# cafferychen777/flashdeconv

Hardware: AMD Instinct MI355X
Metric: spots/sec to convergence (1M x 2000 x 30) (higher is better)
Workload: dtype f64

## Files before the change

### flashdeconv_amd/csrc/tile_kernels.cpp

```cpp
#include "fdx_env.h"
#include <algorithm>
#include <cmath>
#include <cstdlib>
#include <memory>
#include <mutex>

#include "fdx_internal.h"
#include "fdx_kernels.h"
#include "sketch_plan.h"
#include "tile_device.h"
#include "tile_plan.h"
#include "tile_variant.h"

namespace fdx {

struct TilePlanDevice {
    TilePlanHost h;
    DevBuf w, off, len, ent_base, slot_bucket;
    int RS = 0;
    int WB = 0;
    size_t lds = 0;
};

const double* log_table_dev(hipStream_t st) {
    static std::mutex mu;
    static double* tabs[64] = {};
    int dev = 0;
    if (hipGetDevice(&dev) != hipSuccess || dev < 0 || dev >= 64) return nullptr;
    std::lock_guard<std::mutex> lock(mu);
    if (!tabs[dev]) {
        std::vector<double> t((size_t)LOG_TAB_N);
        for (int i = 0; i < LOG_TAB_N; ++i) {
            const unsigned bits = (unsigned)(LOG_TAB_BASE + i) << LOG_TAB_SHIFT;
            float c;
            std::memcpy(&c, &bits, 4);
            t[(size_t)i] = (double)(-logl((long double)c) + (long double)LOG_TAB_EXP_SHIFT * 0.693147180559945309417232121458176568L);
        }
        double* p = nullptr;
        if (hipMalloc(&p, t.size() * sizeof(double)) != hipSuccess) return nullptr;
        if (hipMemcpyAsync(p, t.data(), t.size() * sizeof(double), hipMemcpyHostToDevice, st) != hipSuccess ||
            hipStreamSynchronize(st) != hipSuccess) {
            (void)hipFree(p);
            return nullptr;
        }
        tabs[dev] = p;
    }
    return tabs[dev];
}

static thread_local bool t_f64_math = false;
TileF64Math::TileF64Math(bool on) : prev(t_f64_math) { t_f64_math = on; }
TileF64Math::~TileF64Math() { t_f64_math = prev; }

static int tile_logv() {
    if (t_f64_math) return 0;
    const char* e = fdx::env("FDX_TILE_LOGV");
    return e ? atoi(e) : 2;
}

static bool tile_cfg(int dtype, int mode, int K, int d, int logv, TileVariant* out) {
    if ((dtype != FDX_F32 && dtype != FDX_F64) || K < 1 || K > 64 || d < 1) return false;
    if (mode != FDX_PRE_RAW && mode != FDX_PRE_LOG_CPM && mode != FDX_PRE_LOG_CPM_SPARSE) return false;
    const bool raw = mode == FDX_PRE_RAW;
    TileVariant v = raw ? TileVariant{12, 4, 11} : TileVariant{16, 0, 8};
    v.TT = (K + 15) / 16;
    if (K > 32 || d > 4 * v.NWC * v.JW) {
        v = raw ? TileVariant{12, 4, 22, 4, true} : TileVariant{8, 0, 32, 4, true};
        if (d > 4 * v.NWC * v.JW) return false;
    }
    v.logv = (dtype == FDX_F32 && !raw && logv != 0) ? 2 : 0;
    v.avl2 = v.wide || (!raw && v.logv == 0);
    v.wg = v.wide && raw;
    *out = v;
    return true;
}

static size_t tile_lds_bytes(int RS, int NE, int mode, int WB = 0) {
    const size_t NEp = ((size_t)NE + 7) & ~(size_t)7;
    const size_t below = 2 * ((size_t)WB + (size_t)TILE_ROWS * RS) + NEp * (WB ? 2 : 10) + 2 * TILE_ROWS * (8 + 4);
    if (mode == FDX_PRE_RAW) return below;
    return below <= (size_t)LOG_TAB_LDS ? (size_t)160 * 1024 : (size_t)161 * 1024;
}

static const TilePlanDevice* tile_plan_for(const SketchPlan& sp, int dtype, int mode, const TileVariant& v, hipStream_t st) {
    const int sz = dtype == FDX_F32 ? 4 : 8;
    const int key = ((dtype == FDX_F32 ? 0 : 1) * 2 + (mode != FDX_PRE_RAW ? 1 : 0)) * 3 + (v.wide ? 2 : v.TT - 1);
    static_assert(SketchPlan::kTileKeys == 12, "key space of the schedules: input type x raw / log x {one tile, two tiles, wide}");
    std::lock_guard<std::mutex> lock(sp.tile_mu);
    if (sp.tile_tried[key]) return sp.tile[key].get();
    sp.tile_tried[key] = true;
    const bool dbg = fdx::env("FDX_DEBUG") != nullptr;
    if (!sp.scatter_ok || sp.host_bucket.empty()) return nullptr;
    const size_t red_bytes = tile_red_bytes(v.NWC, v.avl2, v.TT);
    const int unit = (v.wide ? 128 : 1024) / sz;
    std::unique_ptr<TilePlanDevice> best;
    int GB0 = (int)round_up(sp.G, unit);
    while ((size_t)(v.wg ? round_up((GB0 + 1) * 8, 16) : 0) + (size_t)TILE_ROWS * (GB0 * sz + TILE_ROW_PAD) < red_bytes) GB0 += unit;
    for (int GB = GB0; GB >= unit; GB -= unit) {
        const int RS = GB * sz + TILE_ROW_PAD;
        const int WB = v.wg ? (int)round_up((GB + 1) * 8, 16) : 0;
        if ((size_t)WB + (size_t)TILE_ROWS * RS < red_bytes) break;
        if (tile_lds_bytes(RS, sp.G, mode, WB) > 160 * 1024) continue;
        auto cand = std::make_unique<TilePlanDevice>();
        if (!build_tile_plan(sp.host_bucket.data(), sp.host_w.data(), sp.G, sp.d, v.NWC, v.JW, GB, &cand->h)) return nullptr;
        cand->RS = RS;
        cand->WB = WB;
        cand->lds = tile_lds_bytes(RS, cand->h.NE, mode, WB);
        if (dbg) std::fprintf(stderr, "[fdx] tile plan: G=%d d=%d waves=%d+%d GB=%d blocks=%d NE=%d steps=%d lds=%zu\n", sp.G, sp.d, v.NWC,
                              v.NWL, GB, cand->h.NBLK, cand->h.NE, cand->h.steps, cand->lds);
        if (cand->lds > 160 * 1024) continue;
        best = std::move(cand);
        break;
    }
    if (!best) return nullptr;
    TilePlanDevice& t = *best;
    auto up = [&](DevBuf& b, const void* src, size_t bytes) -> int {
        FDX_TRY(b.alloc(bytes));
        FDX_TRY(copy_h2d(b.p, src, bytes, st));
        return 0;
    };
    const int jp = JW_PAD(v.JW);
    std::vector<unsigned char> len_pad((size_t)v.NWC * t.h.NBLK * jp + 16, 0);
    for (int wv = 0; wv < v.NWC; ++wv)
        for (int c = 0; c < t.h.NBLK; ++c)
            for (int j = 0; j < v.JW; ++j)
                len_pad[((size_t)wv * t.h.NBLK + c) * jp + j] = t.h.len[((size_t)wv * t.h.NBLK + c) * v.JW + j];
    std::vector<double> wg_tab;
    if (t.WB) {
        const int per = t.WB / 8;
        wg_tab.assign((size_t)t.h.NBLK * per, 0.0);
        for (int g = 0; g < sp.G; ++g)
            if (sp.host_bucket[(size_t)g] >= 0) wg_tab[(size_t)(g / t.h.GB) * per + g % t.h.GB] = sp.host_w[(size_t)g];
        for (size_t i = 0; i < t.h.off.size(); ++i)
            if (t.h.gene[i] < 0) t.h.off[i] = (unsigned short)t.h.GB;
    }
    if ((t.WB ? up(t.w, wg_tab.data(), wg_tab.size() * 8) : up(t.w, t.h.w.data(), t.h.w.size() * 8)) ||
        up(t.off, t.h.off.data(), t.h.off.size() * 2) || up(t.len, len_pad.data(), len_pad.size()) || up(t.ent_base, t.h.ent_base.data(), t.h.ent_base.size() * 4) ||
        up(t.slot_bucket, t.h.slot_bucket.data(), t.h.slot_bucket.size() * 4))
        return nullptr;
    if (hipStreamSynchronize(st) != hipSuccess) return nullptr;
    sp.tile[key] = std::move(best);
    return sp.tile[key].get();
}

__global__ void tile_xa_kernel(const double* __restrict__ Xs, const int* __restrict__ slot_bucket, int K, int d, int n_groups,
                               int TT, double* __restrict__ XA) {
    const int i = blockIdx.x * blockDim.x + threadIdx.x;
    if (i >= n_groups * TT * 64) return;
    const int lane = i & 63, t = (i >> 6) % TT, wj = (i >> 6) / TT;
    const int b = slot_bucket[wj * 4 + (lane >> 4)];
    const int type = t * 16 + (lane & 15);
    XA[i] = (b >= 0 && type < K) ? Xs[(size_t)type * d + b] : 0.0;
}

bool tile_sketch_ok(int dtype, long long ldy, const void* Y, int G, int d, int K, int mode, const SketchPlanDev& plan,
                    hipStream_t st) {
    if (!plan.owner) return false;
    TileVariant v;
    if (G <= 0 || !tile_cfg(dtype, mode, K, d, tile_logv(), &v)) return false;
    const int sz = dtype == FDX_F32 ? 4 : 8;
    if ((K > 32 || d > 512) && fdx::env("FDX_NO_TILE_WIDE")) return false;
    if (((size_t)G * sz) % 16 != 0 || ((size_t)ldy * sz) % 16 != 0 || (reinterpret_cast<uintptr_t>(Y) & 15) != 0) return false;
    return tile_plan_for(*plan.owner, dtype, mode, v, st) != nullptr;
}

int launch_tile_sketch(const void* Y, int dtype, long long ldy, const int* row_map, long long n, int G, int d, int mode,
                       const SketchPlanDev& plan, const double* Xs, int K, double* H, long long ldh, double* row_sumsq,
                       hipStream_t st) {
    if (n <= 0) return 0;
    TileVariant v;
    const TilePlanDevice* t = plan.owner && tile_cfg(dtype, mode, K, d, tile_logv(), &v) ? tile_plan_for(*plan.owner, dtype, mode, v, st) : nullptr;
    if (!t) return fail(FDX_ERR_INVALID, "tile sketch: no schedule for this shape");
    const void* kern = dtype == FDX_F32 ? tile_kernel<float>(mode, v) : tile_kernel<double>(mode, v);
    if (!kern) {
        char msg[128];
        std::snprintf(msg, sizeof msg, "tile sketch: no kernel for dtype %d mode %d, waves %d + %d x %d, TT %d, AVL2 %d, LOGV %d, WG %d",
                      dtype, mode, v.NWC, v.NWL, v.JW, v.TT, (int)v.avl2, v.logv, (int)v.wg);
        return fail(FDX_ERR_INVALID, msg);
    }
    TileArgs a{};
    a.ldy = ldy; a.n = n; a.ldh = ldh; a.G = G; a.d = d; a.K = K;
    a.NE = t->h.NE; a.GB = t->h.GB; a.NBLK = t->h.NBLK; a.RS = t->RS; a.jw_used = t->h.jw_used; a.WB = t->WB;
    const double* w_tab = t->w.as<double>();
    const unsigned short* off_tab = t->off.as<unsigned short>();
    const unsigned char* len_tab = t->len.as<unsigned char>();
    const int* ent_base = t->ent_base.as<int>();
    const int* slot_bucket = t->slot_bucket.as<int>();
    const double* log_tab = nullptr;
    if (mode != FDX_PRE_RAW) {
        log_tab = log_table_dev(st);
        if (!log_tab) return fail(FDX_ERR_HIP, "tile sketch: log table upload failed");
    }
    const long long n_tiles = (n + TILE_ROWS - 1) / TILE_ROWS;
    const int grid = (int)std::min<long long>(n_tiles, 256);
    DevBuf xa;
    const double* XA = nullptr;
    if (v.avl2) {
        const int n_groups = v.NWC * v.JW;
        FDX_TRY(xa.alloc((size_t)n_groups * v.TT * 64 * sizeof(double)));
        hipLaunchKernelGGL(tile_xa_kernel, dim3(ceil_div((long long)n_groups * v.TT * 64, 256)), dim3(256), 0, st, Xs, slot_bucket, K, d,
                           n_groups, v.TT, xa.as<double>());
        FDX_CHECK_LAUNCH();
        XA = xa.as<double>();
    }
    if (t->lds > 64 * 1024) FDX_HIP(hipFuncSetAttribute(kern, hipFuncAttributeMaxDynamicSharedMemorySize, (int)t->lds));
    void* args[] = {(void*)&a, (void*)&Y, (void*)&row_map, (void*)&Xs, (void*)&H, (void*)&row_sumsq, (void*)&w_tab, (void*)&off_tab,
                    (void*)&len_tab, (void*)&ent_base, (void*)&slot_bucket, (void*)&log_tab, (void*)&XA};
    FDX_HIP(hipLaunchKernel(kern, dim3(grid), dim3((v.NWC + v.NWL) * 64), args, t->lds, st));
    return 0;
}

bool fused_sketch_contract_ok(int dtype, long long ldy, const void* Y, int G, int d, int K, int mode, const SketchPlanDev& plan,
                              hipStream_t st) {
    if (fdx::env("FDX_NO_FUSED")) return false;
    return tile_sketch_ok(dtype, ldy, Y, G, d, K, mode, plan, st);
}

int launch_sketch_contract(const void* Y, int dtype, long long ldy, const int* row_map, long long n, int G, int d, int mode,
                           const SketchPlanDev& plan, const double* Xs, int K, double* H, long long ldh, double* row_sumsq,
                           hipStream_t st) {
    if (n <= 0) return 0;
    if (!tile_sketch_ok(dtype, ldy, Y, G, d, K, mode, plan, st)) return fail(FDX_ERR_INVALID, "sketch -> H: no one-kernel form for this shape");
    return launch_tile_sketch(Y, dtype, ldy, row_map, n, G, d, mode, plan, Xs, K, H, ldh, row_sumsq, st);
}

}

namespace fdx {
__global__ void log1p_f32_probe_kernel(const float* __restrict__ y, float scale, long long n, float* __restrict__ out) {
    const long long i = (long long)blockIdx.x * blockDim.x + threadIdx.x;
    if (i < n) out[i] = tile_log1p_f32(y[i], scale);
}
}

extern "C" int fdx_log1p_f32(const float* y, float scale, int64_t n, float* out) {
    using namespace fdx;
    FDX_REQUIRE(n >= 0 && (n == 0 || (y && out)), "fdx_log1p_f32: null argument");
    if (n == 0) return 0;
    DevBuf in, res;
    FDX_TRY(in.alloc((size_t)n * 4));
    FDX_TRY(res.alloc((size_t)n * 4));
    FDX_HIP(hipMemcpy(in.p, y, (size_t)n * 4, hipMemcpyHostToDevice));
    hipLaunchKernelGGL(log1p_f32_probe_kernel, dim3((unsigned)ceil_div(n, 256)), dim3(256), 0, nullptr, in.as<float>(), scale,
                       (long long)n, res.as<float>());
    FDX_CHECK_LAUNCH();
    FDX_HIP(hipMemcpy(out, res.p, (size_t)n * 4, hipMemcpyDeviceToHost));
    return 0;
}

extern "C" int fdx_tile_schedule(const int32_t* gene_bucket, const double* gene_w, int32_t G, int32_t d, int32_t NW,
                                   int32_t JW, int32_t GB, int32_t* dims_out ,
                                   int32_t* slot_bucket_out, uint8_t* len_out, int32_t* ent_base_out, double* w_out,
                                   uint16_t* off_out, int64_t cap_entries) {
    using namespace fdx;
    FDX_REQUIRE(gene_bucket && gene_w && dims_out, "fdx_tile_schedule: null argument");
    TilePlanHost h;
    FDX_REQUIRE(build_tile_plan(gene_bucket, gene_w, G, d, NW, JW, GB, &h), "fdx_tile_schedule: shape cannot be scheduled");
    dims_out[0] = h.NBLK; dims_out[1] = h.NE; dims_out[2] = h.steps; dims_out[3] = h.max_wave_steps;
    if (!slot_bucket_out) return 0;
    FDX_REQUIRE(len_out && ent_base_out && w_out && off_out && cap_entries >= h.NE, "fdx_tile_schedule: output too small");
    std::copy(h.slot_bucket.begin(), h.slot_bucket.end(), slot_bucket_out);
    std::copy(h.len.begin(), h.len.end(), len_out);
    std::copy(h.ent_base.begin(), h.ent_base.end(), ent_base_out);
    std::copy(h.w.begin(), h.w.end(), w_out);
    std::copy(h.off.begin(), h.off.end(), off_out);
    return 0;
}

extern "C" int fdx_sketch_path(int32_t y_dtype, const void* Y_dev, int64_t ldy, int32_t G, int32_t d, int32_t K, int32_t mode_y_in,
                               const int32_t* bucket, const double* weight_y, int32_t* path_out,
                               int32_t* dims_out ) {
    using namespace fdx;
    FDX_REQUIRE(bucket && weight_y && path_out, "fdx_sketch_path: null argument");
    FDX_REQUIRE(G > 0 && K > 0 && d > 0 && ldy >= G, "fdx_sketch_path: bad shape");
    const int32_t mode_y = mode_y_in & 0xff;
    if (dims_out) std::fill(dims_out, dims_out + 6, 0);
    hipStream_t st = nullptr;
    PoolStream pool_stream(st);
    std::shared_ptr<SketchPlan> plan;
    FDX_TRY(sketch_plan_cached(bucket, weight_y, G, d, st, &plan));
    *path_out = 0;
    if (!fused_sketch_contract_ok(y_dtype, ldy, Y_dev, G, d, K, mode_y, plan->dev(), st)) return 0;
    TileVariant v;
    const TilePlanDevice* t = tile_cfg(y_dtype, mode_y, K, d, tile_logv(), &v) ? tile_plan_for(*plan, y_dtype, mode_y, v, st) : nullptr;
    FDX_REQUIRE(t != nullptr, "fdx_sketch_path: the one-kernel form was accepted without a schedule");
    *path_out = v.wide ? 2 : 1;
    if (dims_out) {
        dims_out[0] = v.NWC; dims_out[1] = v.NWL; dims_out[2] = v.JW; dims_out[3] = v.TT;
        dims_out[4] = t->h.GB; dims_out[5] = t->h.NBLK;
    }
    return 0;
}
```

### flashdeconv_amd/csrc/tile_plan.cpp

```cpp
#include "tile_plan.h"

#include <algorithm>
#include <numeric>

namespace fdx {

bool build_tile_plan(const int* gene_bucket, const double* gene_w, int G, int d, int NW, int JW, int GB, TilePlanHost* out) {
    if (G <= 0 || d <= 0 || NW <= 0 || JW <= 0 || GB <= 0 || GB > 65536) return false;
    const int n_groups = NW * JW;
    if (d > 4 * n_groups) return false;
    const int NBLK = (G + GB - 1) / GB;
    TilePlanHost& p = *out;
    p = TilePlanHost();
    p.G = G; p.d = d; p.NW = NW; p.JW = JW; p.GB = GB; p.NBLK = NBLK;

    std::vector<std::vector<int>> genes((size_t)d);
    for (int g = 0; g < G; ++g) {
        const int b = gene_bucket[g];
        if (b < 0) continue;
        if (b >= d) return false;
        genes[(size_t)b].push_back(g);
    }
    std::vector<int> cnt((size_t)d * NBLK, 0);
    for (int b = 0; b < d; ++b)
        for (int g : genes[(size_t)b]) cnt[(size_t)b * NBLK + g / GB]++;

    struct Group { int b[4]; int cost; std::vector<int> len; };
    std::vector<Group> groups((size_t)n_groups);
    std::vector<int> total((size_t)d, 0);
    for (int b = 0; b < d; ++b) total[(size_t)b] = (int)genes[(size_t)b].size();
    std::vector<char> used((size_t)d, 0);
    int n_left = d;
    for (int gi = 0; gi < n_groups; ++gi) {
        Group& gr = groups[(size_t)gi];
        gr.len.assign((size_t)NBLK, 0);
        gr.cost = 0;
        for (int q = 0; q < 4; ++q) gr.b[q] = -1;
        for (int q = 0; q < 4 && n_left > 0; ++q) {
            int best = -1, best_inc = 0;
            for (int b = 0; b < d; ++b) {
                if (used[(size_t)b]) continue;
                int inc = 0;
                for (int c = 0; c < NBLK; ++c) inc += std::max(0, cnt[(size_t)b * NBLK + c] - gr.len[(size_t)c]);
                if (q == 0) inc = -total[(size_t)b];
                if (best < 0 || inc < best_inc || (inc == best_inc && total[(size_t)b] > total[(size_t)best])) {
                    best = b;
                    best_inc = inc;
                }
            }
            used[(size_t)best] = 1;
            --n_left;
            gr.b[q] = best;
            for (int c = 0; c < NBLK; ++c) gr.len[(size_t)c] = std::max(gr.len[(size_t)c], cnt[(size_t)best * NBLK + c]);
        }
        for (int c = 0; c < NBLK; ++c) {
            if (gr.len[(size_t)c] > 255) return false;
            gr.cost += gr.len[(size_t)c];
        }
    }
    std::vector<int> gorder((size_t)n_groups);
    std::iota(gorder.begin(), gorder.end(), 0);
    std::stable_sort(gorder.begin(), gorder.end(), [&](int a, int b) { return groups[(size_t)a].cost > groups[(size_t)b].cost; });
    std::vector<std::vector<int>> of_wave((size_t)NW);
    std::vector<int> load((size_t)NW, 0);
    for (int gi : gorder) {
        int best = -1;
        for (int w = 0; w < NW; ++w)
            if ((int)of_wave[(size_t)w].size() < JW && (best < 0 || load[(size_t)w] < load[(size_t)best])) best = w;
        of_wave[(size_t)best].push_back(gi);
        load[(size_t)best] += groups[(size_t)gi].cost;
    }

    p.slot_bucket.assign((size_t)n_groups * 4, -1);
    p.len.assign((size_t)NW * NBLK * JW, 0);
    p.ent_base.assign((size_t)NW * (NBLK + 1), 0);
    p.w.clear();
    p.off.clear();
    p.gene.clear();
    for (int w = 0; w < NW; ++w) {
        int wave_steps = 0;
        for (int j = 0; j < JW; ++j)
            for (int q = 0; q < 4; ++q) {
                const int b = groups[(size_t)of_wave[(size_t)w][(size_t)j]].b[q];
                p.slot_bucket[((size_t)w * JW + j) * 4 + q] = b;
                if (b >= 0) p.jw_used = std::max(p.jw_used, j + 1);
            }
        std::vector<int> taken((size_t)JW * 4, 0);
        for (int c = 0; c < NBLK; ++c) {
            p.ent_base[(size_t)w * (NBLK + 1) + c] = (int)p.w.size();
            for (int j = 0; j < JW; ++j) {
                const Group& gr = groups[(size_t)of_wave[(size_t)w][(size_t)j]];
                const int L = gr.len[(size_t)c];
                p.len[((size_t)w * NBLK + c) * JW + j] = (unsigned char)L;
                wave_steps += L;
                for (int t = 0; t < L; ++t)
                    for (int q = 0; q < 4; ++q) {
                        double wt = 0.0;
                        int o = 0;
                        int gid = -1;
                        const int b = gr.b[q];
                        if (b >= 0) {
                            int& k = taken[(size_t)j * 4 + q];
                            const std::vector<int>& L_b = genes[(size_t)b];
                            if (k < (int)L_b.size() && L_b[(size_t)k] / GB == c) {
                                wt = gene_w[L_b[(size_t)k]];
                                o = L_b[(size_t)k] - c * GB;
                                gid = L_b[(size_t)k];
                                ++k;
                            }
                        }
                        p.w.push_back(wt);
                        p.off.push_back((unsigned short)o);
                        p.gene.push_back(gid);
                    }
            }
        }
        p.ent_base[(size_t)w * (NBLK + 1) + NBLK] = (int)p.w.size();
        for (int q = 0; q < 8; ++q) {
            p.w.push_back(0.0);
            p.off.push_back(0);
            p.gene.push_back(-1);
        }
        p.steps += wave_steps;
        p.max_wave_steps = std::max(p.max_wave_steps, wave_steps);
        for (int j = 0; j < JW; ++j)
            for (int q = 0; q < 4; ++q) {
                const int b = groups[(size_t)of_wave[(size_t)w][(size_t)j]].b[q];
                if (b >= 0 && taken[(size_t)j * 4 + q] != (int)genes[(size_t)b].size()) return false;
            }
    }
    p.NE = (int)p.w.size();
    return true;
}

}
```

### flashdeconv_amd/csrc/tile_plan.h

```cpp
#pragma once
#include <vector>

namespace fdx {

struct TilePlanHost {
    int G = 0, d = 0, NW = 0, JW = 0, GB = 0, NBLK = 0;
    int NE = 0;
    int steps = 0;
    int max_wave_steps = 0;
    int jw_used = 0;
    std::vector<int> slot_bucket;
    std::vector<unsigned char> len;
    std::vector<int> ent_base;
    std::vector<double> w;
    std::vector<unsigned short> off;
    std::vector<int> gene;
};

bool build_tile_plan(const int* gene_bucket, const double* gene_w, int G, int d, int NW, int JW, int GB, TilePlanHost* out);


}
```

Measured before the change: 279.0 million.

## Assign bucket groups to waves by per-block critical path with swap refinement

```diff
diff --git a/flashdeconv_amd/csrc/tile_kernels.cpp b/flashdeconv_amd/csrc/tile_kernels.cpp
--- a/flashdeconv_amd/csrc/tile_kernels.cpp
+++ b/flashdeconv_amd/csrc/tile_kernels.cpp
@@ -106,8 +106,8 @@
         cand->RS = RS;
         cand->WB = WB;
         cand->lds = tile_lds_bytes(RS, cand->h.NE, mode, WB);
-        if (dbg) std::fprintf(stderr, "[fdx] tile plan: G=%d d=%d waves=%d+%d GB=%d blocks=%d NE=%d steps=%d lds=%zu\n", sp.G, sp.d, v.NWC,
-                              v.NWL, GB, cand->h.NBLK, cand->h.NE, cand->h.steps, cand->lds);
+        if (dbg) std::fprintf(stderr, "[fdx] tile plan: G=%d d=%d waves=%d+%d GB=%d blocks=%d NE=%d steps=%d crit_steps=%d lds=%zu\n", sp.G, sp.d, v.NWC,
+                              v.NWL, GB, cand->h.NBLK, cand->h.NE, cand->h.steps, cand->h.crit_steps, cand->lds);
         if (cand->lds > 160 * 1024) continue;
         best = std::move(cand);
         break;
diff --git a/flashdeconv_amd/csrc/tile_plan.cpp b/flashdeconv_amd/csrc/tile_plan.cpp
--- a/flashdeconv_amd/csrc/tile_plan.cpp
+++ b/flashdeconv_amd/csrc/tile_plan.cpp
@@ -61,15 +61,80 @@
     std::vector<int> gorder((size_t)n_groups);
     std::iota(gorder.begin(), gorder.end(), 0);
     std::stable_sort(gorder.begin(), gorder.end(), [&](int a, int b) { return groups[(size_t)a].cost > groups[(size_t)b].cost; });
+    std::vector<int> wave_of((size_t)n_groups, 0), n_of((size_t)NW, 0);
+    std::vector<int> L((size_t)NW * NBLK, 0);
+    std::vector<int> top((size_t)NBLK * 3), top_w((size_t)NBLK * 3);
+    auto refresh_top = [&]() {
+        for (int c = 0; c < NBLK; ++c) {
+            int* t = &top[(size_t)c * 3];
+            int* tw = &top_w[(size_t)c * 3];
+            t[0] = t[1] = t[2] = 0;
+            tw[0] = tw[1] = tw[2] = -1;
+            for (int w = 0; w < NW; ++w) {
+                int v = L[(size_t)w * NBLK + c], vw = w;
+                for (int k = 0; k < 3; ++k)
+                    if (tw[k] < 0 || v > t[k]) { std::swap(v, t[k]); std::swap(vw, tw[k]); }
+            }
+        }
+    };
+    auto max_without = [&](int c, int u, int v) {
+        for (int k = 0; k < 3; ++k) {
+            const int w = top_w[(size_t)c * 3 + k];
+            if (w >= 0 && w != u && w != v) return top[(size_t)c * 3 + k];
+        }
+        return 0;
+    };
+    for (int gi : gorder) {
+        const std::vector<int>& len = groups[(size_t)gi].len;
+        refresh_top();
+        int best = -1;
+        long long best_crit = 0, best_sq = 0;
+        for (int w = 0; w < NW; ++w) {
+            if (n_of[(size_t)w] >= JW) continue;
+            long long crit = 0, sq = 0;
+            for (int c = 0; c < NBLK; ++c) {
+                const int was = L[(size_t)w * NBLK + c], now = was + len[(size_t)c];
+                crit += std::max(max_without(c, w, w), now);
+                sq += (long long)now * now - (long long)was * was;
+            }
+            if (best < 0 || crit < best_crit || (crit == best_crit && sq < best_sq)) { best = w; best_crit = crit; best_sq = sq; }
+        }
+        wave_of[(size_t)gi] = best;
+        n_of[(size_t)best]++;
+        for (int c = 0; c < NBLK; ++c) L[(size_t)best * NBLK + c] += len[(size_t)c];
+    }
+    refresh_top();
+    for (int pass = 0, moved = 1; moved && pass < 64; ++pass) {
+        moved = 0;
+        for (int ga = 0; ga < n_groups; ++ga)
+            for (int gb = ga + 1; gb < n_groups; ++gb) {
+                const int u = wave_of[(size_t)ga], v = wave_of[(size_t)gb];
+                if (u == v) continue;
+                const std::vector<int>& la = groups[(size_t)ga].len;
+                const std::vector<int>& lb = groups[(size_t)gb].len;
+                long long d_crit = 0, d_sq = 0;
+                for (int c = 0; c < NBLK; ++c) {
+                    const int diff = lb[(size_t)c] - la[(size_t)c];
+                    if (diff == 0) continue;
+                    const int lu = L[(size_t)u * NBLK + c], lv = L[(size_t)v * NBLK + c];
+                    d_crit += std::max(max_without(c, u, v), std::max(lu + diff, lv - diff)) - top[(size_t)c * 3];
+                    d_sq += (long long)(lu + diff) * (lu + diff) + (long long)(lv - diff) * (lv - diff) - (long long)lu * lu - (long long)lv * lv;
+                }
+                if (d_crit > 0 || (d_crit == 0 && d_sq >= 0)) continue;
+                for (int c = 0; c < NBLK; ++c) {
+                    const int diff = lb[(size_t)c] - la[(size_t)c];
+                    L[(size_t)u * NBLK + c] += diff;
+                    L[(size_t)v * NBLK + c] -= diff;
+                }
+                wave_of[(size_t)ga] = v;
+                wave_of[(size_t)gb] = u;
+                refresh_top();
+                moved = 1;
+            }
+    }
     std::vector<std::vector<int>> of_wave((size_t)NW);
-    std::vector<int> load((size_t)NW, 0);
-    for (int gi : gorder) {
-        int best = -1;
-        for (int w = 0; w < NW; ++w)
-            if ((int)of_wave[(size_t)w].size() < JW && (best < 0 || load[(size_t)w] < load[(size_t)best])) best = w;
-        of_wave[(size_t)best].push_back(gi);
-        load[(size_t)best] += groups[(size_t)gi].cost;
-    }
+    for (int gi : gorder) of_wave[(size_t)wave_of[(size_t)gi]].push_back(gi);
+    for (int c = 0; c < NBLK; ++c) p.crit_steps += top[(size_t)c * 3];
 
     p.slot_bucket.assign((size_t)n_groups * 4, -1);
     p.len.assign((size_t)NW * NBLK * JW, 0);
diff --git a/flashdeconv_amd/csrc/tile_plan.h b/flashdeconv_amd/csrc/tile_plan.h
--- a/flashdeconv_amd/csrc/tile_plan.h
+++ b/flashdeconv_amd/csrc/tile_plan.h
@@ -8,6 +8,7 @@
     int NE = 0;
     int steps = 0;
     int max_wave_steps = 0;
+    int crit_steps = 0;
     int jw_used = 0;
     std::vector<int> slot_bucket;
     std::vector<unsigned char> len;
```

Result: no change. 276.7 million (-0.8%).
